# bowang-lab/BioReason

Hardware: AMD Instinct MI355X
Metric: GRPO samples/sec (NT-500M+Qwen3-1.7B, DNA 2x1024, prompt 2180, gen 256) (higher is better)
Workload: dtype bf16

## Files before the change

bioreason_amd/csrc/k_gemm.hip:

```cpp
#include <type_traits>

#include "bra_device.h"
#include "bra_api_internal.h"

namespace bra {

enum : int {
    EPI_BF16 = 0,
    EPI_F32 = 1,
    EPI_LSE = 2,
    EPI_DLOGIT = 3,
    EPI_ATOMIC = 4,
    EPI_SWIGLU = 5,
};

struct GemmArgs {
    const bf16_t* A;  long lda;
    const bf16_t* B;  long ldb;
    const bf16_t* A2; long lda2;
    const bf16_t* B2; long ldb2;
    void* C;          long ldc;
    int M, N, K, K2;
    float alpha;
    const bf16_t* bias;
    const bf16_t* res;
    long ldres;
    int accumulate;
    int split_k;
    const int* tgt;
    float* part_max;
    float* part_sum;
    float* tgt_logit;
    const float* lse;
    const float* coef;
    int nchunk;
    int swiglu_F;
};

template <int BK>
__device__ __forceinline__ int swz_chunk(int row, int c) {
    return BK == 64 ? (c ^ (row & 7)) : (c ^ ((row >> 2) & 3));
}

#ifdef BRA_EMU
__device__ __forceinline__ void epi_pin(u32x2&) {}
#else
__device__ __forceinline__ void epi_pin(u32x2& v) { asm volatile("" : "+v"(v)); }
#endif
template <bool BIAS>
__device__ __forceinline__ float epi_scale_bias(float a, float alpha, float b) {
    float t = a * alpha;
// ... 903 lines not shown
    int t = 0;
    for (; t + LOOK < nt; ++t) body(t, std::true_type{});
    for (; t < nt; ++t) body(t, std::false_type{});
    auto epi_group = [&](auto HC) {
        constexpr int hcol = decltype(HC)::value;
        gemm_epilogue_w<EPI, WM>(g, *reinterpret_cast<f32x4 (*)[4][WM]>(&acc[4 * hcol]), m0 + wm * (16 * WM), n0 + wn * (16 * WN) + 64 * hcol, lane,
                                 smem + wave * (16 * WM * EPI_RS));
    };
    epi_group(std::integral_constant<int, 0>{});
    if constexpr (WN / 4 > 1) epi_group(std::integral_constant<int, 1>{});
    static_assert(WN / 4 <= 2, "two 64-column groups per wave at most");
}

constexpr int SWG_RS = 80;
__device__ __forceinline__ float silu_epi(float x) { return x / (1.f + __expf(-x)); }
__device__ __forceinline__ void ring_epilogue_swiglu(const GemmArgs& g, f32x4 (&acc)[4][8], int mw0, int f0, int lane, char* lw) {
    const int fr = lane & 15, fq = lane >> 4;
    const float alpha = g.alpha;
    char* wp = lw + fr * SWG_RS + 8 * fq;
#pragma unroll
    for (int mi = 0; mi < 8; ++mi)
#pragma unroll
        for (int j = 0; j < 2; ++j) {
            float v[4];
#pragma unroll
            for (int r = 0; r < 4; ++r) {
                const float gb = round_bf(acc[2 * j][mi][r] * alpha), ub = round_bf(acc[2 * j + 1][mi][r] * alpha);
                v[r] = round_bf(silu_epi(gb)) * ub;
            }
            u32x2 o; o.x = pack_bf2(v[0], v[1]); o.y = pack_bf2(v[2], v[3]);
            st8(wp + mi * (16 * SWG_RS) + j * 32, o);
        }
    wave_lds_sync();
    sched_fence();
    const int rrow = lane >> 2, rch = lane & 3;
    const char* rdp = lw + rrow * SWG_RS + 16 * rch;
    bf16_t* cp = (bf16_t*)g.C + ((long)(mw0 + rrow) * g.ldc + f0 + 8 * rch);
    const long cstep = 16 * g.ldc;
    const bool full = mw0 + 128 <= g.M;
#pragma unroll
    for (int jj = 0; jj < 8; ++jj) {
        const u32x4 xv = ld16(rdp + jj * (16 * SWG_RS));
        if (full || mw0 + rrow + 16 * jj < g.M) st16(cp + jj * cstep, xv);
    }
}

template <int EPI, int PH2 = 0>
__global__ __launch_bounds__(512, 2) void gemm_ring_kernel(GemmArgs g) {
    constexpr int BM = 256, BN = 256, BK = 64, HALF = 128 * BK * 2, NSLOT = 10;
    BRA_DYN_SMEM(smem);
    const int tid = (int)threadIdx.x;
    const int lane = tid & 63, wave = uniform_i(tid >> 6);
    const int wr = wave >> 2, wc = wave & 3;

    const int tiles_m = (g.M + BM - 1) / BM, tiles_n = (g.N + BN - 1) / BN;
    const int ntiles = tiles_m * tiles_n;
    int bid = (int)blockIdx.x;
    int kslice = 0;
// ... 13 lines not shown
    if (EPI == EPI_ATOMIC && g.split_k > 1) {
        int per = (kt_end + g.split_k - 1) / g.split_k;
        kt_begin = kslice * per;
        kt_end = kt_begin + per < kt_end ? kt_begin + per : kt_end;
        if (kt_begin >= kt_end) return;
    }
    const int nt = kt_end - kt_begin;
    const int nstream = 4 * nt;

    const int prow = lane >> 3, lchunk = ((lane & 7) ^ (lane >> 3)) * 8;
    int rowB[4], rowA[4];
#pragma unroll
    for (int i = 0; i < 4; ++i) {
        const int loc = (i >> 1) * 128 + wave * 16 + (i & 1) * 8 + prow;
        int rb = n0 + loc;
        if (EPI == EPI_SWIGLU) rb = tile_n * 128 + (loc >> 5) * 16 + (loc & 15) + ((loc & 16) ? g.swiglu_F : 0);
        rowB[i] = rb < g.N ? rb : g.N - 1;
        int ra = m0 + loc; rowA[i] = ra < g.M ? ra : g.M - 1;
    }
    const bf16_t* src[8];
    auto src_init = [&](int h, int kt) {
        const bool main = kt < nk1;
        const long kcol = (long)(main ? kt : kt - nk1) * BK + lchunk;
#pragma unroll
        for (int pc = 0; pc < 2; ++pc) {
            if (h < 2) src[h * 2 + pc] = (main ? g.B : g.B2) + kcol + (long)rowB[h * 2 + pc] * (main ? g.ldb : g.ldb2);
            else src[h * 2 + pc] = (main ? g.A : g.A2) + kcol + (long)rowA[(h - 2) * 2 + pc] * (main ? g.lda : g.lda2);
        }
    };
#pragma unroll
    for (int h = 0; h < 4; ++h) src_init(h, kt_begin);
// ... 66 lines not shown
        for (int t = 0; t < nt; ++t) {
            const int sB = wrap(rb2 + (wc >> 1)), sA = wrap(rb2 + 2 + wr);
            read_b(sB, I0{}); read_b(sB, I1{}); sched_fence(); read_a(sA, 0);
            issue(t + 1, I2{}, wrap(rb2 + 6)); issue(t + 1, I3{}, wrap(rb2 + 7)); wait2(gp); ++gp;
            sched_fence(); bare_barrier(); wait_lds(); sched_fence();
            mma(I0{}, I0{}); mma(I0{}, I1{});
            sched_fence(); bare_barrier();
            read_a(sA, 1);
            issue(t + 2, I0{}, wrap(rb2 + 8)); issue(t + 2, I1{}, wrap(rb2 + 9)); wait2(gp); ++gp;
            sched_fence(); bare_barrier(); wait_lds(); sched_fence();
            mma(I1{}, I1{}); mma(I1{}, I0{});
            sched_fence(); bare_barrier();
            rb2 = rb2 + 4 >= NSLOT ? rb2 + 4 - NSLOT : rb2 + 4;
        }
        if (wr == 0) bare_barrier();
        if constexpr (EPI == EPI_SWIGLU) ring_epilogue_swiglu(g, acc, m0 + wr * 128, tile_n * 128 + wc * 32, lane, smem + wave * (128 * SWG_RS));
        else gemm_epilogue_w<EPI, 8>(g, acc, m0 + wr * 128, n0 + wc * 64, lane, smem + wave * (128 * EPI_RS));
        return;
    }
    issue(0, I0{}, 0); issue(0, I1{}, 1); issue(0, I2{}, 2); issue(0, I3{}, 3);
    issue(1, I0{}, 4); issue(1, I1{}, 5); issue(1, I2{}, 6);
    wait_phase(-1);
    bare_barrier();
    if (wr == 1) bare_barrier();
    int rbase = 0;
    int gph = 0;
#pragma unroll 1
    for (int t = 0; t < nt; ++t) {
        const int sB = wrap(rbase + (wc >> 1)), sA = wrap(rbase + 2 + wr);
        read_b(sB, I0{}); sched_fence(); read_a(sA, 0);
        issue(t + 1, I3{}, wrap(rbase + 7)); wait_phase(gph); ++gph;
// ... 6 lines not shown
        mma(I0{}, I1{});
        sched_fence(); bare_barrier();
        read_a(sA, 1);
        issue(t + 2, I1{}, wrap(rbase + 9)); wait_phase(gph); ++gph;
        sched_fence(); bare_barrier(); wait_lds(); sched_fence();
        mma(I1{}, I1{});
        sched_fence(); bare_barrier();
        issue(t + 2, I2{}, rbase); wait_phase(gph); ++gph;
        sched_fence(); bare_barrier(); sched_fence();
        mma(I1{}, I0{});
        sched_fence(); bare_barrier();
        rbase = rbase + 4 >= NSLOT ? rbase + 4 - NSLOT : rbase + 4;
    }
    if (wr == 0) bare_barrier();

    if constexpr (EPI == EPI_SWIGLU) ring_epilogue_swiglu(g, acc, m0 + wr * 128, tile_n * 128 + wc * 32, lane, smem + wave * (128 * SWG_RS));
    else gemm_epilogue_w<EPI, 8>(g, acc, m0 + wr * 128, n0 + wc * 64, lane, smem + wave * (128 * EPI_RS));
}

template <int OUTF32>
__global__ __launch_bounds__(256) void gemm_skinny_kernel(GemmArgs g) {
    __shared__ float red[4][64][4];
    const int tid = (int)threadIdx.x, lane = tid & 63, wave = tid >> 6;
    const int fr = lane & 15, fq = lane >> 4;
    const int n0 = (int)blockIdx.x * 16;
    int rn = n0 + fr; rn = rn < g.N ? rn : g.N - 1;
    int rm = fr < g.M ? fr : g.M - 1;
    f32x4 acc = {0.f, 0.f, 0.f, 0.f};
    {
        const bf16_t* wp = g.B + (long)rn * g.ldb + fq * 8;
        const bf16_t* xp = g.A + (long)rm * g.lda + fq * 8;
// ... 328 lines not shown

extern "C" int bra_gemm_swiglu_bf16_nt(const void* A, long lda, const void* W, long ldw, const void* A2, long lda2, const void* B2, long ldb2,
                                       int K2, void* C, long ldc, int M, int F, int K, float alpha, void* stream) {
    if (M == 0 || F == 0) return 0;
    GemmArgs g = {};
    g.A = (const bf16_t*)A; g.lda = lda; g.B = (const bf16_t*)W; g.ldb = ldw;
    g.A2 = (const bf16_t*)A2; g.lda2 = lda2; g.B2 = (const bf16_t*)B2; g.ldb2 = ldb2;
    g.C = C; g.ldc = ldc; g.M = M; g.N = 2 * F; g.K = K; g.K2 = K2; g.alpha = alpha; g.swiglu_F = F;
    int e = check_common(g);
    if (e) return e;
    if (!C || ldc % 8 || ((size_t)C & 15)) return BRA_ERR_ARG;
    if (K % 64 || K2 % 64 || F % 128 || M <= 16) return BRA_ERR_UNSUPPORTED;
    return launch_ring<EPI_SWIGLU>(g, (bra_stream_t)stream);
}

extern "C" int bra_gemm_bf16_nt_splitk(const void* A, long lda, const void* B, long ldb, void* C, long ldc, int M,
                                       int N, int K, float alpha, int split_k, void* stream) {
    GemmArgs g = {};
    g.A = (const bf16_t*)A; g.lda = lda; g.B = (const bf16_t*)B; g.ldb = ldb;
    g.C = C; g.ldc = ldc; g.M = M; g.N = N; g.K = K; g.alpha = alpha; g.split_k = split_k < 1 ? 1 : split_k;
    if (M == 0 || N == 0) return 0;
    int e = check_common(g);
    if (e) return e;
    if (!C) return BRA_ERR_ARG;
    return dispatch_bk<EPI_ATOMIC>(g, (bra_stream_t)stream);
}

extern "C" int bra_lmhead_lse_partials(const void* H, long ldh, const void* E, long lde, int M, int V, int K,
                                       const int* tgt, float* part_max, float* part_sum, float* tgt_logit,
                                       void* stream) {
// ... 26 lines not shown
```

bioreason_amd/csrc/k_norm.hip:

```cpp
#include "bra_device.h"
#include "bra_api_internal.h"

namespace bra {

__global__ __launch_bounds__(256) void rmsnorm_fwd_kernel(const bf16_t* x, long ldx, const bf16_t* w, bf16_t* y,
                                                          long ldy, float* rstd_out, int rows, int cols, float eps) {
    const int row = (int)blockIdx.x * 4 + (int)(threadIdx.x >> 6);
    const int lane = lane_id();
    const bool live = row < rows;
    const bf16_t* xr = x + (long)(live ? row : 0) * ldx;
    float ss = 0.f;
    for (int c = lane * 8; c < cols; c += 512) {
        float f[8];
        unpack8(ld16(xr + c), f);
#pragma unroll
        for (int i = 0; i < 8; ++i) ss += f[i] * f[i];
    }
    ss = wave_sum<64>(ss);
    const float rstd = rsqrtf(ss / (float)cols + eps);
    if (!live) return;
    if (rstd_out && lane == 0) rstd_out[row] = rstd;
    bf16_t* yr = y + (long)row * ldy;
    for (int c = lane * 8; c < cols; c += 512) {
        float f[8], g[8];
// ... 277 lines not shown
    }
    float o[8];
#pragma unroll
    for (int i = 0; i < 8; ++i) {
        const float other = wave_shfl_xor(x[i], LPH / 2);
        const float c = i < 4 ? c0[i & 3] : c1[i & 3], sn = i < 4 ? s0[i & 3] : s1[i & 3];
        o[i] = (is_q || is_k) ? (upper ? x[i] * c + other * sn : x[i] * c - other * sn) : x[i];
    }
    if (!live) return;
    const int b = t / a.S, sidx = t % a.S;
    bf16_t* dst;
    if (is_q) dst = a.q + b * a.q_sb + sidx * a.q_ss + (long)h * a.q_sh;
    else if (is_k) dst = a.k + b * a.k_sb + (sidx + a.s_off) * a.k_ss + (long)(h - a.Hq) * a.k_sh;
    else dst = a.v + b * a.v_sb + (sidx + a.s_off) * a.v_ss + (long)(h - a.Hq - a.Hkv) * a.v_sh;
    st16(dst + j * 8, pack8(o));
}

template <int HD>
__global__ __launch_bounds__(256) void qk_norm_rope_bwd_vec_kernel(RopeBwdArgs a) {
    constexpr int LPH = HD / 8, HALF = HD / 2;
    const int H = a.Hq + 2 * a.Hkv;
    const long nhead = (long)a.T * H;
    const long gl = (long)blockIdx.x * 256 + threadIdx.x;
    const long hidx = gl / LPH;
    const int j = (int)(gl % LPH);
    const bool live = hidx < nhead;
    const long hc = live ? hidx : nhead - 1;
    const int h = (int)(hc % H);
    const int t = (int)(hc / H);
    const bool is_q = h < a.Hq, is_k = !is_q && h < a.Hq + a.Hkv;
// ... 113 lines not shown
                  hd, eps, qscale, (bf16_t*)q, q_sb, q_ss, q_sh, (bf16_t*)k, k_sb, k_ss, k_sh, (bf16_t*)v, v_sb,
                  v_ss, v_sh, s_off};
    const long total = (long)T * (Hq + 2 * Hkv) * (hd / 2);
    const bool vec = (hd == 128 || hd == 64) && ldqkv % 8 == 0 && !((q_sb | q_ss | q_sh | k_sb | k_ss | k_sh | v_sb | v_ss | v_sh) & 7);
    if (vec) {
        const long lanes = (long)T * (Hq + 2 * Hkv) * (hd / 8);
        const dim3 grid((unsigned)((lanes + 255) / 256));
        if (hd == 128) BRA_LAUNCH((qk_norm_rope_fwd_vec_kernel<128>), grid, dim3(256), 0, stream, a);
        else BRA_LAUNCH((qk_norm_rope_fwd_vec_kernel<64>), grid, dim3(256), 0, stream, a);
        return BRA_LAUNCH_STATUS();
    }
    BRA_LAUNCH(qk_norm_rope_fwd_kernel, dim3((unsigned)((total + 255) / 256)), dim3(256), 0, stream, a);
    return BRA_LAUNCH_STATUS();
}

extern "C" int bra_qk_norm_rope_bwd(const void* qkv, long ldqkv, const void* qw, const void* kw, const float* cosT,
                                    const float* sinT, const int* pos, int T, int S, int Hq, int Hkv, int hd,
                                    float eps, float qscale, const void* dq, long q_sb, long q_ss, long q_sh,
                                    const void* dk, long k_sb, long k_ss, long k_sh, const void* dv, long v_sb,
                                    long v_ss, long v_sh, void* dqkv, long lddqkv, void* stream) {
    if (T == 0) return 0;
    if (!qkv || !cosT || !sinT || !pos || !dq || !dk || !dv || !dqkv || S <= 0 || T % S) return BRA_ERR_ARG;
    if (!pow2(hd) || hd < 2 || hd > 128) return BRA_ERR_UNSUPPORTED;
    RopeBwdArgs a = {(const bf16_t*)qkv, ldqkv, (const bf16_t*)qw, (const bf16_t*)kw, cosT, sinT, pos, T, S, Hq,
                     Hkv, hd, eps, qscale, (const bf16_t*)dq, q_sb, q_ss, q_sh, (const bf16_t*)dk, k_sb, k_ss, k_sh,
                     (const bf16_t*)dv, v_sb, v_ss, v_sh, (bf16_t*)dqkv, lddqkv};
    const long total = (long)T * (Hq + 2 * Hkv) * (hd / 2);
    const bool vec = (hd == 128 || hd == 64) && ldqkv % 8 == 0 && lddqkv % 8 == 0 &&
                     !((q_sb | q_ss | q_sh | k_sb | k_ss | k_sh | v_sb | v_ss | v_sh) & 7);
    if (vec) {
// ... 10 lines not shown
```

bioreason_amd/engine.py:

```python
from __future__ import annotations

import math
from dataclasses import dataclass, field
from typing import Dict, List, Optional, Tuple

import torch

from . import ops
from .arena import TrainableArena

BF16 = torch.bfloat16


def rope_tables(npos: int, hd: int, theta: float, device, round_bf16: bool = True) -> Tuple[torch.Tensor, torch.Tensor]:
    inv = 1.0 / (theta ** (torch.arange(0, hd, 2, dtype=torch.float32) / hd))
    fr = torch.arange(npos, dtype=torch.float32)[:, None] * inv[None, :]
    c, s = fr.cos(), fr.sin()
    if round_bf16:
        c, s = c.to(BF16).float(), s.to(BF16).float()
    return c.contiguous().to(device), s.contiguous().to(device)


class LoraGroup:

# ... 68 lines not shown


def _mix32(a: int, b: int) -> int:
    h = (a * 0x9E3779B1 + b * 0x85EBCA6B + 0x165667B1) & 0xFFFFFFFF
    h ^= h >> 15
    h = (h * 0x2C1B3C6D) & 0xFFFFFFFF
    h ^= h >> 12
    h = (h * 0x297A2D39) & 0xFFFFFFFF
    h ^= h >> 15
    return h


import contextlib as _contextlib
import os as _os
FUSE_SWIGLU = _os.environ.get("BRA_FUSE_SWIGLU", "1") == "1"

_nullctx = _contextlib.nullcontext

LORA_GROUP_INDEX = {"qkv": 0, "o": 1, "gu": 2, "d": 3}


def lora_drop_seeds(pass_seed: int, layer: int, group: str, n_targets: int):
    base = (layer * 4 + LORA_GROUP_INDEX[group]) * 4
    return [_mix32(pass_seed, base + j) for j in range(n_targets)]


class QwenEngine:
    def __init__(self, cfg, device):
        self.cfg = cfg
        self.device = device
# ... 96 lines not shown

    def _layer_fwd_fp8(self, li: int, x: torch.Tensor, m: SeqMeta, kv_out, R):
        L = self.layers[li]
        B, S, T = m.B, m.S, m.B * m.S
        cosT, sinT = self.rope(m.max_pos or m.S)
        xq, xs = ops.quant_rows_fp8(x, rms_eps=self.eps)
        qkv = ops.gemm_fp8_nt(xq, xs, R["Wqkv"][0], R["Wqkv"][1])
        q = torch.empty((B, S, self.Hq, self.hd), dtype=BF16, device=x.device)
        if kv_out is None:
            k = torch.empty((B, S, self.Hkv, self.hd), dtype=BF16, device=x.device)
            v = torch.empty((B, S, self.Hkv, self.hd), dtype=BF16, device=x.device)
            s_off = 0
        else:
            kc, vc, s_off = kv_out[:3]
            k, v = kc.permute(0, 2, 1, 3), vc.permute(0, 2, 1, 3)
        ops.qk_norm_rope_fwd(qkv, L.qn, L.kn, cosT, sinT, m.pos, S, self.Hq, self.Hkv, self.hd, self.eps, 1.0, q, k, v, s_off)
        if kv_out is not None:
            k, v = k[:, :s_off + S], v[:, :s_off + S]
        vt = ops.head_transpose(v)
        if kv_out is not None and len(kv_out) > 3 and kv_out[3] is not None:
            kv_out[3].append(vt)
        o, _ = ops.attn_fwd(q, k, vt, m.kmask, True, self.scale, need_lse=False)
        oq, os_ = ops.quant_rows_fp8(o.view(T, self.Nq))
        h = ops.gemm_fp8_nt(oq, os_, R["Wo"][0], R["Wo"][1], res=x)
        hq, hs = ops.quant_rows_fp8(h, rms_eps=self.eps)
        gu = ops.gemm_fp8_nt(hq, hs, R["Wgu"][0], R["Wgu"][1])
        aq, as_ = ops.swiglu_quant_fp8(gu)
        return ops.gemm_fp8_nt(aq, as_, R["Wd"][0], R["Wd"][1], res=h)

    def layer_fwd(self, li: int, x: torch.Tensor, m: SeqMeta, save: bool, kv_out=None):
        w8 = getattr(self, "_fp8", None)
        if w8 is not None and not save:
            return self._layer_fwd_fp8(li, x, m, kv_out, w8[li]), None
        L = self.layers[li]
        B, S, T = m.B, m.S, m.B * m.S
        cosT, sinT = self.rope(m.max_pos or m.S)
        xn = ops.rmsnorm_fwd(x, L.ln1, self.eps)
        qkv, t1 = self._lora_fwd(xn, L.Wqkv, L.lora["qkv"], m.lora_on, drop=self._drop(m, li, "qkv"))
        q = torch.empty((B, S, self.Hq, self.hd), dtype=BF16, device=x.device)
        if kv_out is None:
            k = torch.empty((B, S, self.Hkv, self.hd), dtype=BF16, device=x.device)
            v = torch.empty((B, S, self.Hkv, self.hd), dtype=BF16, device=x.device)
            s_off = 0
        else:
            kc, vc, s_off = kv_out[:3]
            k, v = kc.permute(0, 2, 1, 3), vc.permute(0, 2, 1, 3)
        ops.qk_norm_rope_fwd(qkv, L.qn, L.kn, cosT, sinT, m.pos, S, self.Hq, self.Hkv, self.hd, self.eps, 1.0, q, k, v, s_off)
        if kv_out is not None:
            k, v = k[:, :s_off + S], v[:, :s_off + S]
        vt = ops.head_transpose(v)
        if kv_out is not None and len(kv_out) > 3 and kv_out[3] is not None:
            kv_out[3].append(vt)
        o, lse = ops.attn_fwd(q, k, vt, m.kmask, True, self.scale, need_lse=save)
        o2 = o.view(T, self.Nq)
        h, t2 = self._lora_fwd(o2, L.Wo, L.lora["o"], m.lora_on, res=x, drop=self._drop(m, li, "o"))
        hn = ops.rmsnorm_fwd(h, L.ln2, self.eps)
        gu = t3 = act = None
        if not save and FUSE_SWIGLU:
            G3, d3 = L.lora["gu"], self._drop(m, li, "gu")
            if G3 is not None and m.lora_on:
                t3 = ops.lora_down_drop(hn, G3.A, G3.scaling, d3[0], d3[1]) if d3 is not None else self._down(hn, G3.A, G3.scaling, len(G3.n_sizes) * G3.r)
                act = ops.gemm_swiglu(hn, L.Wgu, a2=t3, b2=G3.B)
            else:
                act = ops.gemm_swiglu(hn, L.Wgu)
        if act is None:
            if t3 is not None:
                gu = ops.gemm_nt(hn, L.Wgu, a2=t3, b2=L.lora["gu"].B)
            else:
                gu, t3 = self._lora_fwd(hn, L.Wgu, L.lora["gu"], m.lora_on, drop=self._drop(m, li, "gu"))
            act = ops.swiglu_fwd(gu)
        y, t4 = self._lora_fwd(act, L.Wd, L.lora["d"], m.lora_on, res=h, drop=self._drop(m, li, "d"))
        saved = (x, xn, t1, qkv, q, k, v, o, lse, t2, h, hn, t3, gu, act, t4) if save else None
        return y, saved

    def layer_bwd(self, li: int, dy: torch.Tensor, saved, m: SeqMeta, prefix: int = 0, extra_dkv=None):
        L = self.layers[li]
        (x, xn, t1, qkv, q, k, v, o, lse, t2, h, hn, t3, gu, act, t4) = saved
        B, S, T = m.B, m.S, m.B * m.S
        cosT, sinT = self.rope(m.max_pos or m.S)
# ... 146 lines not shown
        n, S = ids32.shape
        T = n * S
        dev = ids32.device
        cosT, sinT = self.rope(S)
        pos = torch.arange(S, dtype=torch.int32, device=dev).repeat(n)
        x = torch.empty((T, self.H), dtype=BF16, device=dev)
        zero_row = torch.zeros((1, self.H), dtype=BF16, device=dev)
        tok_src = (mask_u8.reshape(-1).to(torch.int32) - 1).clamp_(max=0).neg_().sub_(1)
        ops.embed_scatter_fwd(ids32.reshape(-1), tok_src, self.E, zero_row, x)
        for L in self.layers:
            xn = ops.layernorm_fwd(x, L.ln1_w, L.ln1_b, self.eps)
            qkv = ops.gemm_nt(xn, L.Wqkv, bias=L.bqkv)
            q = torch.empty((n, S, self.nh, self.hd), dtype=BF16, device=dev)
            k = torch.empty_like(q)
            v = torch.empty_like(q)
            ops.qk_norm_rope_fwd(qkv, None, None, cosT, sinT, pos, S, self.nh, self.nh, self.hd, 0.0, self.hd ** -0.5, q, k, v, 0)
            vt = ops.head_transpose(v)
            o, _ = ops.attn_fwd(q, k, vt, mask_u8, False, 1.0, need_lse=False)
            x = ops.gemm_nt(o.view(T, self.H), L.Wo, bias=L.bo, res=x)
            xn = ops.layernorm_fwd(x, L.ln2_w, L.ln2_b, self.eps)
            act = ops.gemm_swiglu(xn, L.Wup) if FUSE_SWIGLU else None
            if act is None:
                act = ops.swiglu_fwd(ops.gemm_nt(xn, L.Wup))
            x = ops.gemm_nt(act, L.Wdown, res=x)
        return ops.layernorm_fwd(x, self.lnf_w, self.lnf_b, self.eps)
```

bioreason_amd/ops.py:

```python
from __future__ import annotations

import math
import os
from typing import Optional, Tuple

import torch

from ._lib import current_stream, get_lib

BF16 = torch.bfloat16


def _ld(t: torch.Tensor) -> int:
    assert t.stride(-1) == 1, "last dim must be contiguous"
    return t.stride(-2) if t.dim() >= 2 else t.shape[-1]


def _rows(t: torch.Tensor) -> int:
    return t.numel() // t.shape[-1]


def _as2d(t: torch.Tensor) -> torch.Tensor:
    return t.reshape(-1, t.shape[-1]) if t.dim() != 2 else t

# ... 201 lines not shown
    return y.view(x.shape)


def gemm_swiglu(x: torch.Tensor, W: torch.Tensor, a2: Optional[torch.Tensor] = None, b2: Optional[torch.Tensor] = None) -> Optional[torch.Tensor]:
    M, K = x.shape
    F = W.shape[0] // 2
    K2 = a2.shape[1] if a2 is not None else 0
    if M <= 16 or K % 64 or K2 % 64 or F % 128 or W.shape[0] != 2 * F:
        return None
    act = torch.empty((M, F), dtype=BF16, device=x.device)
    rc = get_lib().call_rc("bra_gemm_swiglu_bf16_nt", x, _ld(x), W, _ld(W), a2, _ld(a2) if a2 is not None else 0, b2,
                           _ld(b2) if b2 is not None else 0, K2, act, _ld(act), M, F, K, 1.0, current_stream(x))
    return None if rc != 0 else act


def swiglu_fwd(gu: torch.Tensor) -> torch.Tensor:
    gu2 = _as2d(gu)
    F = gu2.shape[1] // 2
    act = torch.empty((gu2.shape[0], F), dtype=BF16, device=gu.device)
    get_lib().call("bra_swiglu_fwd", gu2, _ld(gu2), act, _ld(act), gu2.shape[0], F, current_stream(gu))
    return act


def swiglu_bwd(gu: torch.Tensor, dact: torch.Tensor) -> torch.Tensor:
    gu2, d2 = _as2d(gu), _as2d(dact)
    F = gu2.shape[1] // 2
    dgu = torch.empty_like(gu2)
    get_lib().call("bra_swiglu_bwd", gu2, _ld(gu2), d2, _ld(d2), dgu, _ld(dgu), gu2.shape[0], F, current_stream(gu))
    return dgu


def _bsh_strides(t: torch.Tensor) -> Tuple[int, int, int]:
    assert t.dim() == 4 and t.stride(3) == 1
    return t.stride(0), t.stride(1), t.stride(2)


def qk_norm_rope_fwd(qkv, qw, kw, cosT, sinT, pos, S, Hq, Hkv, hd, eps, qscale, q, k, v, s_off=0):
    T = qkv.shape[0]
    get_lib().call("bra_qk_norm_rope_fwd", qkv, _ld(qkv), qw, kw, cosT, sinT, pos, T, S, Hq, Hkv, hd, eps, qscale,
                   q, *_bsh_strides(q), k, *_bsh_strides(k), v, *_bsh_strides(v), s_off, current_stream(qkv))


def qk_norm_rope_bwd(qkv, qw, kw, cosT, sinT, pos, S, Hq, Hkv, hd, eps, qscale, dq, dk, dv):
    T = qkv.shape[0]
    dqkv = torch.empty_like(qkv)
    get_lib().call("bra_qk_norm_rope_bwd", qkv, _ld(qkv), qw, kw, cosT, sinT, pos, T, S, Hq, Hkv, hd, eps, qscale,
                   dq, *_bsh_strides(dq), dk, *_bsh_strides(dk), dv, *_bsh_strides(dv), dqkv, _ld(dqkv), current_stream(qkv))
    return dqkv


def pad64(n: int) -> int:
    return (n + 63) // 64 * 64


def head_transpose(x: torch.Tensor) -> torch.Tensor:
# ... 389 lines not shown
```

include/bioreason_hip.h:

```cpp
#ifndef BIOREASON_HIP_H
#define BIOREASON_HIP_H
#ifdef __cplusplus
extern "C" {
#endif

#define BRA_ERR_ARG (-1)
#define BRA_ERR_UNSUPPORTED (-2)

int bra_gemm_bf16_nt(const void* A, long lda, const void* B, long ldb, const void* A2, long lda2, const void* B2,
                     long ldb2, int K2, void* C, long ldc, int M, int N, int K, float alpha, const void* bias,
                     const void* res, long ldres, int out_f32, int accumulate, void* stream);

int bra_gemm_bf16_nt_splitk(const void* A, long lda, const void* B, long ldb, void* C, long ldc, int M, int N, int K,
                            float alpha, int split_k, void* stream);

int bra_wgrad_tn(const void* Y, long ldy, const void* T, long ldt, float* C, long c_sn, long c_sr, int M, int N, int R,
                 float alpha, int m_chunk, void* stream);

int bra_lora_down_drop(const void* x, long ldx, const void* A, long lda, void* t, long ldt, int M, int K, int R, float alpha,
                       float p, unsigned s0, unsigned s1, unsigned s2, unsigned s3, int nb_live, void* stream);
int bra_lora_down_splitk_plan(int M, int K);
int bra_lora_down_drop_splitk(const void* x, long ldx, const void* A, long lda, void* t, long ldt, int M, int K, int R, float alpha,
                              float p, unsigned s0, unsigned s1, unsigned s2, unsigned s3, int nb_live, float* part, int ksplit,
                              void* stream);
// ... 12 lines not shown
                       const float* lse, const float* coef, void* dlogits, long ldd, void* stream);

int bra_rmsnorm_fwd(const void* x, long ldx, const void* w, void* y, long ldy, float* rstd, int rows, int cols,
                    float eps, void* stream);
int bra_rmsnorm_bwd(const void* dy, long lddy, const void* x, long ldx, const void* w, const void* dres, long lddres,
                    void* dx, long lddx, int rows, int cols, float eps, void* stream);
int bra_layernorm_fwd(const void* x, long ldx, const void* w, const void* b, void* y, long ldy, int rows, int cols,
                      float eps, void* stream);
int bra_swiglu_fwd(const void* gu, long ldgu, void* act, long ldact, int rows, int F, void* stream);
int bra_swiglu_bwd(const void* gu, long ldgu, const void* dact, long lddact, void* dgu, long lddgu, int rows, int F,
                   void* stream);
int bra_qk_norm_rope_fwd(const void* qkv, long ldqkv, const void* qw, const void* kw, const float* cosT,
                         const float* sinT, const int* pos, int T, int S, int Hq, int Hkv, int hd, float eps,
                         float qscale, void* q, long q_sb, long q_ss, long q_sh, void* k, long k_sb, long k_ss,
                         long k_sh, void* v, long v_sb, long v_ss, long v_sh, int s_off, void* stream);
int bra_qk_norm_rope_bwd(const void* qkv, long ldqkv, const void* qw, const void* kw, const float* cosT,
                         const float* sinT, const int* pos, int T, int S, int Hq, int Hkv, int hd, float eps,
                         float qscale, const void* dq, long q_sb, long q_ss, long q_sh, const void* dk, long k_sb,
                         long k_ss, long k_sh, const void* dv, long v_sb, long v_ss, long v_sh, void* dqkv,
                         long lddqkv, void* stream);

int bra_attn_fwd(const void* q, long q_sb, long q_ss, long q_sh, const void* k, long k_sb, long k_ss, long k_sh,
                 const void* vt, long vt_sb, long vt_sh, long vt_sd, void* o, long o_sb, long o_ss, long o_sh,
                 float* lse, const void* kmask, int B, int Hq, int Hkv, int Sq, int Sk, int hd, int causal,
                 int q_off, float scale, void* stream);
int bra_attn_fwd_split(const void* q, long q_sb, long q_ss, long q_sh, const void* k, long k_sb, long k_ss, long k_sh,
                       const void* vt, long vt_sb, long vt_sh, long vt_sd, void* o, long o_sb, long o_ss, long o_sh,
                       float* lse, const void* kmask, int B, int Hq, int Hkv, int Sq, int Sk, int hd, int causal,
                       int q_off, float scale, int nsplit, float* part_o, float* part_ml, void* stream);
int bra_attn_bwd(const void* q, long q_sb, long q_ss, long q_sh, const void* k, long k_sb, long k_ss, long k_sh,
// ... 28 lines not shown
                         float* part_ml, int B, int Hq, int Hkv, int hd, int Smax, int cur_len, float eps, float scale,
                         int chunk_off, int nchunk_tot, const int* t_dev, void* stream);
int bra_dec_gemm2(const void* x, long ldx, const float* ss_in, int nss_in, const void* norm_w, float eps, const void* W,
                  long ldw, const void* res, long ldres, void* out, long ldo, float* ss_out, int nss_out, int M, int N,
                  int K, int act, int out_f32, void* stream);
int bra_dec_gemm2_packed(const void* x, long ldx, const float* ss_in, int nss_in, const void* norm_w, float eps, const void* W,
                         long ldw, const void* res, long ldres, void* out, long ldo, float* ss_out, int nss_out, int M, int N,
                         int K, int act, int out_f32, int packed, void* stream);
int bra_dec_pack_weights_fp8(const void* W, long ldw, int N, int K, int act, int out_f32, const void* norm_w, void* out_q,
                             float* out_scale, void* stream);
int bra_dec_gemm2_fp8(const void* x, long ldx, const float* ss_in, int nss_in, float eps, const void* Wq, const float* wscale,
                      const void* res, long ldres, void* out, long ldo, float* ss_out, int nss_out, int M, int N, int K, int act,
                      int out_f32, int norm_folded, void* stream);
int bra_gemm_swiglu_bf16_nt(const void* A, long lda, const void* W, long ldw, const void* A2, long lda2, const void* B2, long ldb2, int K2,
                            void* C, long ldc, int M, int F, int K, float alpha, void* stream);
int bra_quant_rows_fp8(const void* x, long ldx, int M, int K, const void* colw, void* q, long ldq, float* scale, int rms, float eps,
                       void* stream);
int bra_swiglu_quant_fp8(const void* gu, long ldgu, int M, int F, void* q, long ldq, float* scale, void* stream);
int bra_gemm_fp8_nt(const void* A8, long lda, const float* sa, const void* B8, long ldb, const float* sb, void* C, long ldc, int M, int N,
                    int K, const void* res, long ldres, int out_f32, void* stream);
int bra_dec_pack_weights(const void* W, long ldw, int N, int K, int act, int out_f32, const void* norm_w, void* out, void* stream);
int bra_dec_pack_weights_rows(const void* W, long ldw, int N, int K, int act, int out_f32, const void* norm_w, int rows, void* out,
                              void* stream);
int bra_row_sumsq(const void* x, long ldx, int M, int K, float* ss, int nss, void* stream);
int bra_dec_attn_shared(const void* qkv, long ldqkv, const void* qw, const float* cosT, const float* sinT, const int* pos,
                        const void* kp, long kp_sr, long kp_sh, long kp_ss, const void* vtp, long vt_sr, long vt_sh,
                        long vt_sd, const void* pmask, float* part_o, float* part_ml, int R, int copies, int Hq, int Hkv,
                        int hd, int P, int nchunk_tot, float eps, float scale, const int* t_dev, void* stream);
int bra_dec_attn_both(const void* qkv, long ldqkv, const void* qw, const void* kw, const float* cosT, const float* sinT,
                      const int* pos, const void* kp, long kp_sr, long kp_sh, long kp_ss, const void* vtp, long vt_sr,
// ... 91 lines not shown
```

Measured before the change: 19.58.

## Fuse SwiGLU into gate-up GEMM when saving tape; fuse V transpose into QK-rope

Adds a gate-up GEMM epilogue that writes both the SwiGLU activation and the raw gate/up outputs, so the training forward pass with saved activations no longer needs a separate swiglu kernel over the gu tensor. It also adds a QK-norm/RoPE kernel that transposes V through shared memory and writes the V-transposed layout directly, replacing the separate head_transpose launch when there is no KV offset. Both are on by default through environment flags. The cost is extra epilogue LDS round-trips and stores in the GEMM, plus a heavier rope kernel with a shared-memory tile.

Result: no change. 19.60 (median of 2 runs) (+0.1%).

```diff
diff --git a/bioreason_amd/csrc/k_gemm.hip b/bioreason_amd/csrc/k_gemm.hip
--- a/bioreason_amd/csrc/k_gemm.hip
+++ b/bioreason_amd/csrc/k_gemm.hip
@@ -12,7 +12,9 @@
     EPI_DLOGIT = 3,
     EPI_ATOMIC = 4,
     EPI_SWIGLU = 5,
+    EPI_SWIGLU_GU = 6,
 };
+constexpr bool epi_is_swiglu(int epi) { return epi == EPI_SWIGLU || epi == EPI_SWIGLU_GU; }
 
 struct GemmArgs {
     const bf16_t* A;  long lda;
@@ -35,6 +37,7 @@
     const float* coef;
     int nchunk;
     int swiglu_F;
+    bf16_t* C2; long ldc2;
 };
 
 template <int BK>
@@ -968,10 +971,25 @@
 
 constexpr int SWG_RS = 80;
 __device__ __forceinline__ float silu_epi(float x) { return x / (1.f + __expf(-x)); }
+template <bool GU>
 __device__ __forceinline__ void ring_epilogue_swiglu(const GemmArgs& g, f32x4 (&acc)[4][8], int mw0, int f0, int lane, char* lw) {
     const int fr = lane & 15, fq = lane >> 4;
     const float alpha = g.alpha;
     char* wp = lw + fr * SWG_RS + 8 * fq;
+    const int rrow = lane >> 2, rch = lane & 3;
+    const char* rdp = lw + rrow * SWG_RS + 16 * rch;
+    const bool full = mw0 + 128 <= g.M;
+    auto flush = [&](bf16_t* base, long ld) {
+        wave_lds_sync();
+        sched_fence();
+        bf16_t* cp = base + ((long)(mw0 + rrow) * ld + f0 + 8 * rch);
+        const long cstep = 16 * ld;
+#pragma unroll
+        for (int jj = 0; jj < 8; ++jj) {
+            const u32x4 xv = ld16(rdp + jj * (16 * SWG_RS));
+            if (full || mw0 + rrow + 16 * jj < g.M) st16(cp + jj * cstep, xv);
+        }
+    };
 #pragma unroll
     for (int mi = 0; mi < 8; ++mi)
 #pragma unroll
@@ -985,17 +1003,22 @@
             u32x2 o; o.x = pack_bf2(v[0], v[1]); o.y = pack_bf2(v[2], v[3]);
             st8(wp + mi * (16 * SWG_RS) + j * 32, o);
         }
-    wave_lds_sync();
-    sched_fence();
-    const int rrow = lane >> 2, rch = lane & 3;
-    const char* rdp = lw + rrow * SWG_RS + 16 * rch;
-    bf16_t* cp = (bf16_t*)g.C + ((long)(mw0 + rrow) * g.ldc + f0 + 8 * rch);
-    const long cstep = 16 * g.ldc;
-    const bool full = mw0 + 128 <= g.M;
-#pragma unroll
-    for (int jj = 0; jj < 8; ++jj) {
-        const u32x4 xv = ld16(rdp + jj * (16 * SWG_RS));
-        if (full || mw0 + rrow + 16 * jj < g.M) st16(cp + jj * cstep, xv);
+    flush((bf16_t*)g.C, g.ldc);
+    if constexpr (GU) {
+#pragma unroll
+        for (int h = 0; h < 2; ++h) {
+            wave_lds_sync();
+            sched_fence();
+#pragma unroll
+            for (int mi = 0; mi < 8; ++mi)
+#pragma unroll
+                for (int j = 0; j < 2; ++j) {
+                    const f32x4& a = acc[2 * j + h][mi];
+                    u32x2 o; o.x = pack_bf2(a[0] * alpha, a[1] * alpha); o.y = pack_bf2(a[2] * alpha, a[3] * alpha);
+                    st8(wp + mi * (16 * SWG_RS) + j * 32, o);
+                }
+            flush(g.C2 + (h ? g.swiglu_F : 0), g.ldc2);
+        }
     }
 }
 
@@ -1039,7 +1062,7 @@
     for (int i = 0; i < 4; ++i) {
         const int loc = (i >> 1) * 128 + wave * 16 + (i & 1) * 8 + prow;
         int rb = n0 + loc;
-        if (EPI == EPI_SWIGLU) rb = tile_n * 128 + (loc >> 5) * 16 + (loc & 15) + ((loc & 16) ? g.swiglu_F : 0);
+        if (epi_is_swiglu(EPI)) rb = tile_n * 128 + (loc >> 5) * 16 + (loc & 15) + ((loc & 16) ? g.swiglu_F : 0);
         rowB[i] = rb < g.N ? rb : g.N - 1;
         int ra = m0 + loc; rowA[i] = ra < g.M ? ra : g.M - 1;
     }
@@ -1136,7 +1159,7 @@
             rb2 = rb2 + 4 >= NSLOT ? rb2 + 4 - NSLOT : rb2 + 4;
         }
         if (wr == 0) bare_barrier();
-        if constexpr (EPI == EPI_SWIGLU) ring_epilogue_swiglu(g, acc, m0 + wr * 128, tile_n * 128 + wc * 32, lane, smem + wave * (128 * SWG_RS));
+        if constexpr (epi_is_swiglu(EPI)) ring_epilogue_swiglu<EPI == EPI_SWIGLU_GU>(g, acc, m0 + wr * 128, tile_n * 128 + wc * 32, lane, smem + wave * (128 * SWG_RS));
         else gemm_epilogue_w<EPI, 8>(g, acc, m0 + wr * 128, n0 + wc * 64, lane, smem + wave * (128 * EPI_RS));
         return;
     }
@@ -1173,7 +1196,7 @@
     }
     if (wr == 0) bare_barrier();
 
-    if constexpr (EPI == EPI_SWIGLU) ring_epilogue_swiglu(g, acc, m0 + wr * 128, tile_n * 128 + wc * 32, lane, smem + wave * (128 * SWG_RS));
+    if constexpr (epi_is_swiglu(EPI)) ring_epilogue_swiglu<EPI == EPI_SWIGLU_GU>(g, acc, m0 + wr * 128, tile_n * 128 + wc * 32, lane, smem + wave * (128 * SWG_RS));
     else gemm_epilogue_w<EPI, 8>(g, acc, m0 + wr * 128, n0 + wc * 64, lane, smem + wave * (128 * EPI_RS));
 }
 
@@ -1532,6 +1555,35 @@
     return launch_ring<EPI_SWIGLU>(g, (bra_stream_t)stream);
 }
 
+extern "C" int bra_swiglu_fwd(const void* gu, long ldgu, void* act, long ldact, int rows, int F, void* stream);
+extern "C" int bra_gemm_swiglu_gu_bf16_nt(const void* A, long lda, const void* W, long ldw, const void* A2, long lda2, const void* B2, long ldb2,
+                                          int K2, void* act, long ldact, void* gu, long ldgu, int M, int F, int K, float alpha, void* stream) {
+    if (M == 0 || F == 0) return 0;
+    GemmArgs g = {};
+    g.A = (const bf16_t*)A; g.lda = lda; g.B = (const bf16_t*)W; g.ldb = ldw;
+    g.A2 = (const bf16_t*)A2; g.lda2 = lda2; g.B2 = (const bf16_t*)B2; g.ldb2 = ldb2;
+    g.C = act; g.ldc = ldact; g.M = M; g.N = 2 * F; g.K = K; g.K2 = K2; g.alpha = alpha; g.swiglu_F = F;
+    g.C2 = (bf16_t*)gu; g.ldc2 = ldgu;
+    int e = check_common(g);
+    if (e) return e;
+    if (!act || !gu || ldact % 8 || ldgu % 8 || (((size_t)act | (size_t)gu) & 15)) return BRA_ERR_ARG;
+    if (K % 64 || K2 % 64 || F % 128 || M <= 16) return BRA_ERR_UNSUPPORTED;
+    const int m1 = ring_split_rows(g);
+    if (m1 > 0) {
+        GemmArgs g2 = g;
+        g.M = m1;
+        g2.M = M - m1;
+        g2.A = g.A + (long)m1 * lda;
+        if (g.A2) g2.A2 = g.A2 + (long)m1 * lda2;
+        g2.C = (bf16_t*)gu + (long)m1 * ldgu; g2.ldc = ldgu; g2.C2 = nullptr; g2.swiglu_F = 0;
+        e = launch_glds<EPI_BF16>(g2, (bra_stream_t)stream);
+        if (e) return e;
+        e = bra_swiglu_fwd(g2.C, ldgu, (bf16_t*)act + (long)m1 * ldact, ldact, g2.M, F, stream);
+        if (e) return e;
+    }
+    return launch_ring<EPI_SWIGLU_GU>(g, (bra_stream_t)stream);
+}
+
 extern "C" int bra_gemm_bf16_nt_splitk(const void* A, long lda, const void* B, long ldb, void* C, long ldc, int M,
                                        int N, int K, float alpha, int split_k, void* stream) {
     GemmArgs g = {};
diff --git a/bioreason_amd/csrc/k_norm.hip b/bioreason_amd/csrc/k_norm.hip
--- a/bioreason_amd/csrc/k_norm.hip
+++ b/bioreason_amd/csrc/k_norm.hip
@@ -315,6 +315,95 @@
     else if (is_k) dst = a.k + b * a.k_sb + (sidx + a.s_off) * a.k_ss + (long)(h - a.Hq) * a.k_sh;
     else dst = a.v + b * a.v_sb + (sidx + a.s_off) * a.v_ss + (long)(h - a.Hq - a.Hkv) * a.v_sh;
     st16(dst + j * 8, pack8(o));
+}
+
+struct RopeVtArgs { bf16_t* vt; long sb, sh, pitch; };
+
+template <int HD>
+__global__ __launch_bounds__(256) void qk_norm_rope_fwd_vt_kernel(RopeArgs a, RopeVtArgs t) {
+    constexpr int LPH = HD / 8, HALF = HD / 2, LD = HD + 2;
+    __shared__ bf16_t tile[64 * LD];
+    const int tid = (int)threadIdx.x;
+    const int h = (int)blockIdx.y, b = (int)blockIdx.z;
+    const int p0 = (a.s_off / 64 + (int)blockIdx.x) * 64;
+    const bool is_q = h < a.Hq, is_k = !is_q && h < a.Hq + a.Hkv, is_v = !is_q && !is_k;
+    const bf16_t* nw = is_q ? a.qw : (is_k ? a.kw : nullptr);
+    for (int idx = tid; idx < 64 * LPH; idx += 256) {
+        const int r = idx / LPH, j = idx % LPH;
+        const int s = p0 + r - a.s_off;
+        const bool live = s >= 0 && s < a.S;
+        const int tok = b * a.S + (live ? s : 0);
+        const bool upper = j >= LPH / 2;
+        const int dh = (j & (LPH / 2 - 1)) * 8;
+        float x[8];
+        unpack8(ld16(a.qkv + (long)tok * a.ldqkv + (long)h * HD + j * 8), x);
+        u32x4 nwv = {0u, 0u, 0u, 0u};
+        if (nw) nwv = ld16(nw + j * 8);
+        f32x4 c0 = {1.f, 1.f, 1.f, 1.f}, c1 = c0, s0 = {0.f, 0.f, 0.f, 0.f}, s1 = s0;
+        if (is_q || is_k) {
+            const int p = a.pos[tok];
+            const float* cp = a.cosT + (long)p * HALF + dh;
+            const float* sp = a.sinT + (long)p * HALF + dh;
+            c0 = *reinterpret_cast<const f32x4*>(cp); c1 = *reinterpret_cast<const f32x4*>(cp + 4);
+            s0 = *reinterpret_cast<const f32x4*>(sp); s1 = *reinterpret_cast<const f32x4*>(sp + 4);
+        }
+        float ss = 0.f;
+#pragma unroll
+        for (int i = 0; i < 8; ++i) ss += x[i] * x[i];
+#pragma unroll
+        for (int m = LPH >> 1; m >= 1; m >>= 1) ss += wave_shfl_xor(ss, m);
+        if (nw) {
+            const float rstd = rsqrtf(ss / (float)HD + a.eps);
+            float w[8];
+            unpack8(nwv, w);
+#pragma unroll
+            for (int i = 0; i < 8; ++i) x[i] = round_bf(w[i] * round_bf(x[i] * rstd));
+        }
+        if (is_q && a.qscale != 1.f) {
+#pragma unroll
+            for (int i = 0; i < 8; ++i) x[i] = round_bf(x[i] * a.qscale);
+        }
+        float o[8];
+#pragma unroll
+        for (int i = 0; i < 8; ++i) {
+            const float other = wave_shfl_xor(x[i], LPH / 2);
+            const float c = i < 4 ? c0[i & 3] : c1[i & 3], sn = i < 4 ? s0[i & 3] : s1[i & 3];
+            o[i] = (is_q || is_k) ? (upper ? x[i] * c + other * sn : x[i] * c - other * sn) : x[i];
+        }
+        u32x4 ov = pack8(o);
+        if (live) {
+            bf16_t* dst;
+            if (is_q) dst = a.q + b * a.q_sb + s * a.q_ss + (long)h * a.q_sh;
+            else if (is_k) dst = a.k + b * a.k_sb + (s + a.s_off) * a.k_ss + (long)(h - a.Hq) * a.k_sh;
+            else dst = a.v + b * a.v_sb + (s + a.s_off) * a.v_ss + (long)(h - a.Hq - a.Hkv) * a.v_sh;
+            st16(dst + j * 8, ov);
+        }
+        if (is_v) {
+            if (!live) ov = u32x4{0u, 0u, 0u, 0u};
+            uint32_t* tp = reinterpret_cast<uint32_t*>(&tile[r * LD + j * 8]);
+            tp[0] = ov.x; tp[1] = ov.y; tp[2] = ov.z; tp[3] = ov.w;
+        }
+    }
+    if (!is_v) return;
+    __syncthreads();
+    bf16_t* op = t.vt + b * t.sb + (long)(h - a.Hq - a.Hkv) * t.sh;
+    for (int q = tid; q < HD * 8; q += 256) {
+        const int d = q >> 3, c = q & 7;
+        const int p = p0 + c * 8;
+        if (p + 8 <= a.s_off) continue;
+        bf16_t* dp = op + (long)d * t.pitch + p;
+        if (p >= a.s_off) {
+            uint32_t w[4];
+#pragma unroll
+            for (int i = 0; i < 4; ++i) {
+                const uint32_t lo = tile[(c * 8 + 2 * i) * LD + d], hi = tile[(c * 8 + 2 * i + 1) * LD + d];
+                w[i] = lo | (hi << 16);
+            }
+            st16(dp, u32x4{w[0], w[1], w[2], w[3]});
+        } else {
+            for (int i = a.s_off - p; i < 8; ++i) dp[i] = tile[(c * 8 + i) * LD + d];
+        }
+    }
 }
 
 template <int HD>
@@ -458,6 +547,27 @@
     return BRA_LAUNCH_STATUS();
 }
 
+extern "C" int bra_qk_norm_rope_fwd_vt(const void* qkv, long ldqkv, const void* qw, const void* kw, const float* cosT,
+                                       const float* sinT, const int* pos, int T, int S, int Hq, int Hkv, int hd,
+                                       float eps, float qscale, void* q, long q_sb, long q_ss, long q_sh, void* k,
+                                       long k_sb, long k_ss, long k_sh, void* v, long v_sb, long v_ss, long v_sh,
+                                       int s_off, void* vt, long vt_sb, long vt_sh, long vt_pitch, void* stream) {
+    if (T == 0) return 0;
+    if (!qkv || !cosT || !sinT || !pos || !q || !k || !v || !vt || S <= 0 || T % S || s_off < 0) return BRA_ERR_ARG;
+    if (vt_pitch % 64 || vt_pitch < ((long)(s_off + S + 63) / 64) * 64) return BRA_ERR_ARG;
+    if (hd != 128 && hd != 64) return BRA_ERR_UNSUPPORTED;
+    if (ldqkv % 8 || ((q_sb | q_ss | q_sh | k_sb | k_ss | k_sh | v_sb | v_ss | v_sh | vt_sb | vt_sh) & 7) || ((size_t)vt & 15))
+        return BRA_ERR_UNSUPPORTED;
+    RopeArgs a = {(const bf16_t*)qkv, ldqkv, (const bf16_t*)qw, (const bf16_t*)kw, cosT, sinT, pos, T, S, Hq, Hkv,
+                  hd, eps, qscale, (bf16_t*)q, q_sb, q_ss, q_sh, (bf16_t*)k, k_sb, k_ss, k_sh, (bf16_t*)v, v_sb,
+                  v_ss, v_sh, s_off};
+    RopeVtArgs t = {(bf16_t*)vt, vt_sb, vt_sh, vt_pitch};
+    const dim3 grid((unsigned)((s_off % 64 + S + 63) / 64), (unsigned)(Hq + 2 * Hkv), (unsigned)(T / S));
+    if (hd == 128) BRA_LAUNCH((qk_norm_rope_fwd_vt_kernel<128>), grid, dim3(256), 0, stream, a, t);
+    else BRA_LAUNCH((qk_norm_rope_fwd_vt_kernel<64>), grid, dim3(256), 0, stream, a, t);
+    return BRA_LAUNCH_STATUS();
+}
+
 extern "C" int bra_qk_norm_rope_bwd(const void* qkv, long ldqkv, const void* qw, const void* kw, const float* cosT,
                                     const float* sinT, const int* pos, int T, int S, int Hq, int Hkv, int hd,
                                     float eps, float qscale, const void* dq, long q_sb, long q_ss, long q_sh,
diff --git a/bioreason_amd/engine.py b/bioreason_amd/engine.py
--- a/bioreason_amd/engine.py
+++ b/bioreason_amd/engine.py
@@ -106,6 +106,19 @@
 import contextlib as _contextlib
 import os as _os
 FUSE_SWIGLU = _os.environ.get("BRA_FUSE_SWIGLU", "1") == "1"
+FUSE_SWIGLU_TAPE = _os.environ.get("BRA_FUSE_SWIGLU_TAPE", "1") == "1"
+FUSE_VT = _os.environ.get("BRA_FUSE_VT", "1") == "1"
+
+
+def _qk_rope_vt(qkv, qw, kw, cosT, sinT, pos, S, Hq, Hkv, hd, eps, qscale, q, k, v, s_off):
+    vt = None
+    if FUSE_VT and s_off == 0:
+        vt = ops.qk_norm_rope_fwd_vt(qkv, qw, kw, cosT, sinT, pos, S, Hq, Hkv, hd, eps, qscale, q, k, v, 0)
+    if vt is None:
+        ops.qk_norm_rope_fwd(qkv, qw, kw, cosT, sinT, pos, S, Hq, Hkv, hd, eps, qscale, q, k, v, s_off)
+    k, v = k[:, :s_off + S], v[:, :s_off + S]
+    return k, v, (vt if vt is not None else ops.head_transpose(v))
+
 
 _nullctx = _contextlib.nullcontext
 
@@ -232,10 +245,7 @@
         else:
             kc, vc, s_off = kv_out[:3]
             k, v = kc.permute(0, 2, 1, 3), vc.permute(0, 2, 1, 3)
-        ops.qk_norm_rope_fwd(qkv, L.qn, L.kn, cosT, sinT, m.pos, S, self.Hq, self.Hkv, self.hd, self.eps, 1.0, q, k, v, s_off)
-        if kv_out is not None:
-            k, v = k[:, :s_off + S], v[:, :s_off + S]
-        vt = ops.head_transpose(v)
+        k, v, vt = _qk_rope_vt(qkv, L.qn, L.kn, cosT, sinT, m.pos, S, self.Hq, self.Hkv, self.hd, self.eps, 1.0, q, k, v, s_off)
         if kv_out is not None and len(kv_out) > 3 and kv_out[3] is not None:
             kv_out[3].append(vt)
         o, _ = ops.attn_fwd(q, k, vt, m.kmask, True, self.scale, need_lse=False)
@@ -263,10 +273,7 @@
         else:
             kc, vc, s_off = kv_out[:3]
             k, v = kc.permute(0, 2, 1, 3), vc.permute(0, 2, 1, 3)
-        ops.qk_norm_rope_fwd(qkv, L.qn, L.kn, cosT, sinT, m.pos, S, self.Hq, self.Hkv, self.hd, self.eps, 1.0, q, k, v, s_off)
-        if kv_out is not None:
-            k, v = k[:, :s_off + S], v[:, :s_off + S]
-        vt = ops.head_transpose(v)
+        k, v, vt = _qk_rope_vt(qkv, L.qn, L.kn, cosT, sinT, m.pos, S, self.Hq, self.Hkv, self.hd, self.eps, 1.0, q, k, v, s_off)
         if kv_out is not None and len(kv_out) > 3 and kv_out[3] is not None:
             kv_out[3].append(vt)
         o, lse = ops.attn_fwd(q, k, vt, m.kmask, True, self.scale, need_lse=save)
@@ -281,6 +288,15 @@
                 act = ops.gemm_swiglu(hn, L.Wgu, a2=t3, b2=G3.B)
             else:
                 act = ops.gemm_swiglu(hn, L.Wgu)
+        elif save and FUSE_SWIGLU_TAPE:
+            G3, d3 = L.lora["gu"], self._drop(m, li, "gu")
+            if G3 is not None and m.lora_on:
+                t3 = ops.lora_down_drop(hn, G3.A, G3.scaling, d3[0], d3[1]) if d3 is not None else self._down(hn, G3.A, G3.scaling, len(G3.n_sizes) * G3.r)
+                fused = ops.gemm_swiglu_gu(hn, L.Wgu, a2=t3, b2=G3.B)
+            else:
+                fused = ops.gemm_swiglu_gu(hn, L.Wgu)
+            if fused is not None:
+                gu, act = fused
         if act is None:
             if t3 is not None:
                 gu = ops.gemm_nt(hn, L.Wgu, a2=t3, b2=L.lora["gu"].B)
@@ -457,8 +473,7 @@
             q = torch.empty((n, S, self.nh, self.hd), dtype=BF16, device=dev)
             k = torch.empty_like(q)
             v = torch.empty_like(q)
-            ops.qk_norm_rope_fwd(qkv, None, None, cosT, sinT, pos, S, self.nh, self.nh, self.hd, 0.0, self.hd ** -0.5, q, k, v, 0)
-            vt = ops.head_transpose(v)
+            k, v, vt = _qk_rope_vt(qkv, None, None, cosT, sinT, pos, S, self.nh, self.nh, self.hd, 0.0, self.hd ** -0.5, q, k, v, 0)
             o, _ = ops.attn_fwd(q, k, vt, mask_u8, False, 1.0, need_lse=False)
             x = ops.gemm_nt(o.view(T, self.H), L.Wo, bias=L.bo, res=x)
             xn = ops.layernorm_fwd(x, L.ln2_w, L.ln2_b, self.eps)
diff --git a/bioreason_amd/ops.py b/bioreason_amd/ops.py
--- a/bioreason_amd/ops.py
+++ b/bioreason_amd/ops.py
@@ -239,6 +239,20 @@
     return None if rc != 0 else act
 
 
+def gemm_swiglu_gu(x: torch.Tensor, W: torch.Tensor, a2: Optional[torch.Tensor] = None,
+                   b2: Optional[torch.Tensor] = None) -> Optional[Tuple[torch.Tensor, torch.Tensor]]:
+    M, K = x.shape
+    F = W.shape[0] // 2
+    K2 = a2.shape[1] if a2 is not None else 0
+    if M <= 16 or K % 64 or K2 % 64 or F % 128 or W.shape[0] != 2 * F:
+        return None
+    gu = torch.empty((M, 2 * F), dtype=BF16, device=x.device)
+    act = torch.empty((M, F), dtype=BF16, device=x.device)
+    rc = get_lib().call_rc("bra_gemm_swiglu_gu_bf16_nt", x, _ld(x), W, _ld(W), a2, _ld(a2) if a2 is not None else 0, b2,
+                           _ld(b2) if b2 is not None else 0, K2, act, _ld(act), gu, _ld(gu), M, F, K, 1.0, current_stream(x))
+    return None if rc != 0 else (gu, act)
+
+
 def swiglu_fwd(gu: torch.Tensor) -> torch.Tensor:
     gu2 = _as2d(gu)
     F = gu2.shape[1] // 2
@@ -264,6 +278,19 @@
     T = qkv.shape[0]
     get_lib().call("bra_qk_norm_rope_fwd", qkv, _ld(qkv), qw, kw, cosT, sinT, pos, T, S, Hq, Hkv, hd, eps, qscale,
                    q, *_bsh_strides(q), k, *_bsh_strides(k), v, *_bsh_strides(v), s_off, current_stream(qkv))
+
+
+def qk_norm_rope_fwd_vt(qkv, qw, kw, cosT, sinT, pos, S, Hq, Hkv, hd, eps, qscale, q, k, v, s_off=0, vt=None) -> Optional[torch.Tensor]:
+    T = qkv.shape[0]
+    if hd not in (64, 128):
+        return None
+    if vt is None:
+        vt = torch.empty((T // S, Hkv, hd, pad64(s_off + S)), dtype=BF16, device=qkv.device)
+    assert vt.stride(3) == 1
+    rc = get_lib().call_rc("bra_qk_norm_rope_fwd_vt", qkv, _ld(qkv), qw, kw, cosT, sinT, pos, T, S, Hq, Hkv, hd, eps, qscale,
+                           q, *_bsh_strides(q), k, *_bsh_strides(k), v, *_bsh_strides(v), s_off,
+                           vt, vt.stride(0), vt.stride(1), vt.stride(2), current_stream(qkv))
+    return None if rc != 0 else vt
 
 
 def qk_norm_rope_bwd(qkv, qw, kw, cosT, sinT, pos, S, Hq, Hkv, hd, eps, qscale, dq, dk, dv):
diff --git a/include/bioreason_hip.h b/include/bioreason_hip.h
--- a/include/bioreason_hip.h
+++ b/include/bioreason_hip.h
@@ -50,6 +50,11 @@
                          const float* sinT, const int* pos, int T, int S, int Hq, int Hkv, int hd, float eps,
                          float qscale, void* q, long q_sb, long q_ss, long q_sh, void* k, long k_sb, long k_ss,
                          long k_sh, void* v, long v_sb, long v_ss, long v_sh, int s_off, void* stream);
+int bra_qk_norm_rope_fwd_vt(const void* qkv, long ldqkv, const void* qw, const void* kw, const float* cosT,
+                            const float* sinT, const int* pos, int T, int S, int Hq, int Hkv, int hd, float eps,
+                            float qscale, void* q, long q_sb, long q_ss, long q_sh, void* k, long k_sb, long k_ss,
+                            long k_sh, void* v, long v_sb, long v_ss, long v_sh, int s_off, void* vt, long vt_sb,
+                            long vt_sh, long vt_pitch, void* stream);
 int bra_qk_norm_rope_bwd(const void* qkv, long ldqkv, const void* qw, const void* kw, const float* cosT,
                          const float* sinT, const int* pos, int T, int S, int Hq, int Hkv, int hd, float eps,
                          float qscale, const void* dq, long q_sb, long q_ss, long q_sh, const void* dk, long k_sb,
@@ -108,6 +113,8 @@
                       int out_f32, int norm_folded, void* stream);
 int bra_gemm_swiglu_bf16_nt(const void* A, long lda, const void* W, long ldw, const void* A2, long lda2, const void* B2, long ldb2, int K2,
                             void* C, long ldc, int M, int F, int K, float alpha, void* stream);
+int bra_gemm_swiglu_gu_bf16_nt(const void* A, long lda, const void* W, long ldw, const void* A2, long lda2, const void* B2, long ldb2, int K2,
+                               void* act, long ldact, void* gu, long ldgu, int M, int F, int K, float alpha, void* stream);
 int bra_quant_rows_fp8(const void* x, long ldx, int M, int K, const void* colw, void* q, long ldq, float* scale, int rms, float eps,
                        void* stream);
 int bra_swiglu_quant_fp8(const void* gu, long ldgu, int M, int F, void* q, long ldq, float* scale, void* stream);
```
